# maxilevi/vits.cpp

Hardware: AMD Instinct MI355X
Metric: audio samples/sec end-to-end (ids -> fp32 PCM in HBM), vits-english architecture, batch=64 x 128 ids (higher is better)
Workload: dtype f32; 1 GPU; c3 b64x128 ref-mode f32 predicted-dur | vits-english = MMS-TTS arch, synthetic weights; batch_per_gpu=64, ids_per_utterance=128, parallelism=utterance-sharded x1

## Files before the change

vits.cpp_amd/csrc/abi_ops_common.h:

```cpp
#pragma once
#include <algorithm>
#include <cstdint>
#include <cstring>
#include <memory>
#include <string>
#include <vector>

#include "../../include/vits.h"
#include "abi_internal.h"
#include "engine.h"

namespace vits {
extern thread_local int g_op_out_fill;
extern thread_local int g_op_arith;

inline bool refuse(const std::string& why) {
    set_err(why);
    return false;
}

struct DevMem {
    void* p = nullptr;
    DevMem() = default;
    DevMem(const DevMem&) = delete;
    DevMem& operator=(const DevMem&) = delete;
    ~DevMem() {
        if (p) hipFree(p);
    }
    static bool ok(hipError_t e, const char* what) { return e == hipSuccess || refuse(what); }
    bool alloc(size_t bytes) { return ok(hipMalloc(&p, std::max<size_t>(bytes, 16)), "device allocation failed"); }
    bool fill(size_t bytes, int byte) { return alloc(bytes) && ok(hipMemset(p, byte, std::max<size_t>(bytes, 16)), "device allocation failed"); }
    bool put(const void* h, size_t bytes) { return h ? alloc(bytes) && ok(hipMemcpy(p, h, bytes, hipMemcpyHostToDevice), "device allocation failed") : fill(bytes, 0); }
    bool put_opt(const void* h, size_t bytes) { return !h || put(h, bytes); }
    bool get(void* h, size_t bytes) const { return ok(hipMemcpy(h, p, bytes, hipMemcpyDeviceToHost), "copy back failed"); }
    float* f() const { return static_cast<float*>(p); }
    uint16_t* h() const { return static_cast<uint16_t*>(p); }
    int* i() const { return static_cast<int*>(p); }
};

inline TensorRef tref(float* p, int channels, int stride) {
    TensorRef t;
    t.p = p;
    t.cs = stride;
    t.bs = (int64_t)channels * stride;
    return t;
}
inline bool lens_ok(const int32_t* lens, int batch, int t) {
    for (int b = 0; lens && b < batch; ++b)
        if (lens[b] < 0 || lens[b] > t) return false;
    return true;
}
inline bool shape_lens_ok(const int32_t* lens, int batch, int t, int t_stride) { return batch >= 1 && t >= 1 && t_stride >= t && lens_ok(lens, batch, t); }

inline bool finish(hipError_t e, const std::string& what = "") {
    if (e == hipSuccess) e = hipDeviceSynchronize();
    if (e == hipSuccess) return true;
    set_err(what.empty() ? std::string(hipGetErrorString(e)) : what + ": " + hipGetErrorString(e));
    return false;
}

inline bool stage_rows(DevMem& dst, const float* src, int batch, int rows, int64_t src_pitch, int64_t pitch, const int32_t* lens, int t) {
    std::vector<float> h((size_t)batch * rows * pitch);
    std::memset(h.data(), 0xFF, h.size() * 4);
    for (int b = 0; src && b < batch; ++b)
        for (int c = 0; c < rows; ++c)
            std::memcpy(&h[((size_t)b * rows + c) * pitch], src + ((size_t)b * rows + c) * src_pitch, sizeof(float) * (size_t)(lens ? lens[b] : t));
    return dst.put(h.data(), h.size() * 4);
}
inline bool unstage_rows(const DevMem& src, float* dst, int batch, int rows, int64_t pitch, int64_t dst_pitch, int t) {
    return DevMem::ok(hipMemcpy2D(dst, (size_t)dst_pitch * 4, src.p, (size_t)pitch * 4, (size_t)t * 4, (size_t)batch * rows, hipMemcpyDeviceToHost), "copy back failed");
}
inline bool stage_group8(DevMem& dst, const float* src, int batch, int channels, int64_t src_pitch, int64_t pitch, const int32_t* lens, int t) {
    std::vector<float> h((size_t)batch * channels * pitch);
    std::memset(h.data(), 0xFF, h.size() * 4);
    for (int b = 0; b < batch; ++b)
        for (int c = 0; c < channels; ++c) {
            const float* s = src + ((size_t)b * channels + c) * src_pitch;
            float* g = &h[((size_t)b * channels + (size_t)(c / 8) * 8) * pitch + (c & 7)];
            for (int n = 0, len = lens ? lens[b] : t; n < len; ++n) g[(size_t)n * 8] = s[n];
        }
    return dst.put(h.data(), h.size() * 4);
}
template <class T>
inline bool unstage_group8(const DevMem& src, T* dst, int batch, int channels, int64_t pitch, int64_t dst_pitch, int t) {
    std::vector<T> h((size_t)batch * channels * pitch);
    if (!src.get(h.data(), h.size() * sizeof(T))) return false;
    for (int b = 0; b < batch; ++b)
        for (int c = 0; c < channels; ++c) {
            const T* g = &h[((size_t)b * channels + (size_t)(c / 8) * 8) * pitch + (c & 7)];
            T* d = dst + ((size_t)b * channels + c) * dst_pitch;
            for (int n = 0; n < t; ++n) d[n] = g[(size_t)n * 8];
        }
    return true;
}

struct OpKnobs {
    KernelKnobs k;
    KernelKnobsScope scope;
    OpKnobs() : k(kernel_knobs()), scope(&k) {
        k.no_tile_map = getenv("VITS_NO_TILE_MAP") != nullptr;
        k.tile_map = getenv("VITS_TILE_MAP") != nullptr;
    }
};
struct OpTileMaps {
    TileMapSet set;
    std::vector<std::unique_ptr<DevMem>> mem;
    bool add(const int32_t* len_in, const int32_t* len_out, int batch, int t_in, int t_out, int width, bool convt) {
        const KernelKnobs& kn = kernel_knobs();
        if (kn.no_tile_map || set.find(width, convt)) return true;
        std::vector<int> la(batch, t_in), lb(batch, t_out);
        if (len_in) la.assign(len_in, len_in + batch);
        if (len_out) lb.assign(len_out, len_out + batch);
        if (!kn.tile_map && !tile_map_needed(la.data(), lb.data(), batch, t_in, t_out, width, convt)) return true;
        std::vector<TileEntry> e((size_t)tile_map_count(la.data(), lb.data(), batch, width, convt) + 1);
        const int64_t n = tile_map_fill(la.data(), lb.data(), batch, width, convt, e.data());
        mem.emplace_back(new DevMem);
        if (!mem.back()->put(e.data(), e.size() * sizeof(TileEntry))) return false;
        return set.add(TileMapRef{static_cast<const TileEntry*>(mem.back()->p), (int)n, width, convt}) || refuse("too many tile widths for one length vector");
    }
    bool add_conv(const int32_t* len_in, const int32_t* len_out, int batch, int t_in, int t_out, bool convt) {
        return add(len_in, len_out, batch, t_in, t_out, tile_shape(TILE_128x128).bn(), convt) && add(len_in, len_out, batch, t_in, t_out, tile_shape(TILE_64x256).bn(), convt);
    }
};

struct Conv {
    PackedConv pc;
    DevMem w, wl, w16, b;
};
inline bool upload_conv(Conv& c, const float* w, const float* bias, size_t bias_n, int cout, int cin, int taps, int epi, int ct_stride, int arith, bool l16_always = false) {
    PackedConv& pc = c.pc;
    const ConvPackDims pd = conv_pack_dims(cout, cin, taps, epi, ct_stride);
    pc.cin = cin, pc.cout = cout, pc.kt = pd.kt, pc.epi = epi, pc.ct_stride = ct_stride;
    pc.rows = pd.rows, pc.mtiles_used = pd.mtiles_used, pc.mtiles = pd.mtiles, pc.nchunks = pd.nchunks;
    if (bias) {
        if (!c.b.put(bias, bias_n * 4)) return false;
        pc.bias = c.b.f();
    }
    if (arith != VITS_ARITH_F32) {
        const std::vector<uint16_t> p16 = pack_conv_weights16(w, cout, cin, taps, epi, ct_stride, arith);
        if (!c.w16.put(p16.data(), p16.size() * 2)) return false;
        pc.wp16 = c.w16.h(), pc.bytes16 = (int64_t)p16.size() * 2;
        return true;
    }
    const std::vector<float> packed = pack_conv_weights(w, cout, cin, taps, epi, ct_stride, &pc.rows, &pc.mtiles_used, &pc.mtiles, &pc.nchunks);
    if (!c.w.put(packed.data(), packed.size() * 4)) return false;
    pc.wp = c.w.f(), pc.bytes = (int64_t)packed.size() * 4;
    if (l16_always || conv_lat16_candidate(epi, taps, cin)) {
        const std::vector<float> pl = repack_conv_weights_l16(packed, pc.mtiles, pc.nchunks, pc.kt);
        if (!c.wl.put(pl.data(), pl.size() * 4)) return false;
        pc.wp_l16 = c.wl.f();
    }
    return true;
}

inline size_t group16_bytes(int batch, int cin, int t) { return (size_t)batch * ((cin + 7) / 8 + 1) * round_up(t, 8) * 8 * 2; }
inline hipError_t conv_transparent(const PackedConv& w, const ConvCall& c, int arith, const DevMem& x16, size_t nan_bytes = 0) {
    if (arith == VITS_ARITH_F32) return launch_conv(w, c, nullptr);
    Ref16 r;
    r.p = x16.h(), r.ts = round_up(c.t_in, 8), r.bs = (int64_t)((w.cin + 7) / 8) * r.ts * 8;
    if (nan_bytes && hipMemsetAsync(x16.p, 0xFF, nan_bytes, nullptr) != hipSuccess) return hipErrorUnknown;
    const hipError_t e = launch_to_group16(c.x, c.len_in, c.batch, w.cin, c.t_in, c.pre_act ? c.slope : 1.0f, r, arith, nullptr);
    if (e != hipSuccess) return e;
    Conv16Call q;
    q.x = r, q.len_in = c.len_in, q.len_out = c.len_out, q.spk = c.spk, q.batch = c.batch, q.t_in = c.t_in, q.t_out = c.t_out, q.dil = c.dil, q.pad_l = c.pad_l;
    q.post_act = c.post_act, q.post_slope = c.post_slope, q.scale = c.scale, q.scale_div = c.scale_div, q.ct_crop = c.ct_crop, q.tile = c.tile;
    q.y = c.y, q.res = c.res, q.acc = c.acc;
    return launch_conv16(w, q, arith, nullptr);
}
}
```

vits.cpp_amd/csrc/kernel_common.h:

```cpp
#pragma once

#include <cstdint>

#include "tile_map.h"

#ifdef __HIPCC__
namespace vits {

typedef float floatx16 __attribute__((ext_vector_type(16)));
typedef float float4v __attribute__((ext_vector_type(4)));
typedef float float2v __attribute__((ext_vector_type(2)));
typedef int int4v __attribute__((ext_vector_type(4)));
typedef int int2v __attribute__((ext_vector_type(2)));
typedef _Float16 half8 __attribute__((ext_vector_type(8)));
typedef __bf16 bf16x8 __attribute__((ext_vector_type(8)));
typedef _Float16 half2v __attribute__((ext_vector_type(2)));
typedef __bf16 bf2v __attribute__((ext_vector_type(2)));

template <bool BF>
__device__ __forceinline__ unsigned pack16(float a, float b) {
    float2v f = {a, b};
    if constexpr (BF) return __builtin_bit_cast(unsigned, __builtin_convertvector(f, bf2v));
    else return __builtin_bit_cast(unsigned, __builtin_convertvector(f, half2v));
}
template <bool BF>
__device__ __forceinline__ float unpack16(unsigned short h) {
    if constexpr (BF) return __builtin_bit_cast(float, (unsigned)h << 16);
    else return (float)__builtin_bit_cast(_Float16, h);
}
template <bool BF>
__device__ __forceinline__ floatx16 mfma16(int4v a, int4v b, floatx16 c) {
    if constexpr (BF) return __builtin_amdgcn_mfma_f32_32x32x16_bf16(__builtin_bit_cast(bf16x8, a), __builtin_bit_cast(bf16x8, b), c, 0, 0, 0);
    else return __builtin_amdgcn_mfma_f32_32x32x16_f16(__builtin_bit_cast(half8, a), __builtin_bit_cast(half8, b), c, 0, 0, 0);
}

struct TileCoord {
    int b, t0, len_a, len_b;
};
__device__ __forceinline__ TileCoord tile_coord(const TileEntry* map, int bx, int bz, int bn, const int* len_a, const int* len_b, int max_a, int max_b) {
    TileCoord c;
    if (map) {
        const int4v e = *reinterpret_cast<const int4v*>(map + bx);
        c.b = e.x, c.t0 = e.y, c.len_a = e.z, c.len_b = e.w;
    } else {
        c.b = bz, c.t0 = bx * bn;
        c.len_a = len_a ? len_a[bz] : max_a;
        c.len_b = len_b ? len_b[bz] : max_b;
    }
    return c;
}

__device__ __forceinline__ __amdgpu_buffer_rsrc_t stream_rsrc(const void* base) {
    return __builtin_amdgcn_make_buffer_rsrc(const_cast<void*>(base), 0, 0x7fffffff, 0x00020000);
}
template <typename V>
__device__ __forceinline__ V load_frag(__amdgpu_buffer_rsrc_t wrsrc, int voff, int step, int sbase = 0) {
    return __builtin_bit_cast(V, __builtin_amdgcn_raw_buffer_load_b128(wrsrc, voff, sbase + step * 1024, 0));
}

__device__ __forceinline__ int64_t group_off(int ch0, int ts, int t) { return ((int64_t)(ch0 >> 3) * ts + t) * 8 + (ch0 & 7); }

__device__ __forceinline__ float scale_or_div(float v, float scale, int scale_div) { return scale_div ? v / scale : v * scale; }

__device__ __forceinline__ void group_add_scale(float (&v)[4], float4v a, float scale, int scale_div) {
#pragma unroll
    for (int e = 0; e < 4; ++e) {
        v[e] = a[e] + v[e];
        v[e] = scale_or_div(v[e], scale, scale_div);
    }
}
template <bool BF>
__device__ __forceinline__ void group_store(float (&v)[4], float* yg, int64_t go, uint16_t* y16, int y16_ts, float y16_slope, int ch0, int t) {
    if (yg) *reinterpret_cast<float4v*>(yg + go) = float4v{v[0], v[1], v[2], v[3]};
    if (y16) {
#pragma unroll
        for (int e = 0; e < 4; ++e) v[e] = fmaxf(v[e], v[e] * y16_slope);
        int2v w2;
        w2.x = (int)pack16<BF>(v[0], v[1]);
        w2.y = (int)pack16<BF>(v[2], v[3]);
        *reinterpret_cast<int2v*>(y16 + group_off(ch0, y16_ts, t)) = w2;
    }
}

__device__ __forceinline__ float ggml_table_lookup(const uint16_t* tab, float x) {
    const uint16_t i = __builtin_bit_cast(uint16_t, (_Float16)x);
    return (float)__builtin_bit_cast(_Float16, tab[i]);
}
__device__ __forceinline__ float gelu_erf(float x) { return 0.5f * x * (1.0f + erff(x * 0.70710678118654752440f)); }
__device__ __forceinline__ float gelu_op(float x, const uint16_t* gelu_tab) { return gelu_tab ? ggml_table_lookup(gelu_tab, x) : gelu_erf(x); }

}
#endif
```

vits.cpp_amd/csrc/kernels.h:

```cpp
#pragma once
#include <hip/hip_runtime.h>
#include <hip/hip_ext.h>

#include <algorithm>
#include <atomic>
#include <cstdint>
#include <cstdlib>
#include <string>
#include <vector>

#include "tile_map.h"

struct vits_edges_desc;

namespace vits {

struct KernelKnobs {
    int narrow_tiles = 64;
    int tile128 = 1;
    int min_blocks = 0;
    bool no_narrow = false;
    int narrow_k1 = 1 << 30;
    int nbuf = 0;
    bool no_oneshot = false;
    int db_min = 1;
    int t16_tile0 = 0;
    bool no_convt16s = false;
    bool convt16s_all = false;
    bool no_convt16l = false;
    bool no_att_lat = false;
    bool att_valu = false;
    int att_nw = 0;
    int att_short = 512;
    int ln_tw = 32;
    bool rbb_c128 = true;
    int rbb_c64k11 = -1;
    int rbb_stream_tiles = -1;
    int rbb_stream_min_blocks = 1536;
    int fuse16_maxc = 256;
    bool fuse32_c128 = true;
    int wn16_ncw = 1;
    int flow_ncw = 2;
    int convt16_r128 = 0;
    int convt16_split_max = 64;
    bool no_rbb_group3_c64 = false;
    bool no_rbb_group3 = false;
    bool no_rb_sum3_f32 = false;
    bool rb_sum3_in_order = false;
    bool rb_sum3_block_only = false;
    bool no_rb_sum3 = false;
    int rb16_narrow_max = 128;
    int flow_narrow_max = 96;
    bool no_ln_fuse = false;
    bool no_dds_lat = false;
    int dds_lat_max_blocks = 96;
    bool no_dp_det_fuse = false;
    int dp_det_lat_max_blocks = 96;
    int lat16h_group_shape = 21;
    bool no_lat16h_group = false;
    bool no_lat16h_pre = false;
    bool no_lat16h = false;
    int lat16h_max_tiles = 2048;
    int lat16h_max_tiles_c128 = 0;
    int lat16h_shape = 21;
    bool no_lat16 = false;
    int lat16_max_waves = 768;
    bool no_tile_map = false;
    bool tile_map = false;
    static KernelKnobs from_env() {
        KernelKnobs k;
        auto num = [](const char* name, int& v) {
            if (const char* e = getenv(name)) v = atoi(e);
        };
        auto flag = [](const char* name, bool& v) { v = getenv(name) != nullptr; };
        num("VITS_NARROW_TILES", k.narrow_tiles);
        flag("VITS_NO_DDS_LAT", k.no_dds_lat);
        flag("VITS_NO_LN_FUSE", k.no_ln_fuse);
        flag("VITS_NO_RB_SUM3", k.no_rb_sum3);
        flag("VITS_RB_SUM3_BLOCK_ONLY", k.rb_sum3_block_only);
        flag("VITS_RB_SUM3_IN_ORDER", k.rb_sum3_in_order);
        flag("VITS_NO_RB_SUM3_F32", k.no_rb_sum3_f32);
        flag("VITS_NO_RBB_GROUP3", k.no_rbb_group3);
        flag("VITS_NO_RBB_GROUP3_C64", k.no_rbb_group3_c64);
        num("VITS_DDS_LAT_MAX_BLOCKS", k.dds_lat_max_blocks);
        flag("VITS_NO_DP_DET_FUSE", k.no_dp_det_fuse);
        num("VITS_DP_DET_LAT_MAX_BLOCKS", k.dp_det_lat_max_blocks);
        num("VITS_TILE128", k.tile128);
        num("VITS_MIN_BLOCKS", k.min_blocks);
        flag("VITS_NO_NARROW", k.no_narrow);
        num("VITS_NARROW_K1", k.narrow_k1);
        num("VITS_NBUF", k.nbuf);
        flag("VITS_NO_ONESHOT", k.no_oneshot);
        num("VITS_DB_MIN", k.db_min);
        num("VITS_T16_TILE0", k.t16_tile0);
        flag("VITS_NO_CONVT16S", k.no_convt16s);
        flag("VITS_CONVT16S_ALL", k.convt16s_all);
        flag("VITS_NO_CONVT16L", k.no_convt16l);
        flag("VITS_ATT_VALU", k.att_valu);
        flag("VITS_NO_ATT_LAT", k.no_att_lat);
        num("VITS_ATT_NW", k.att_nw);
        num("VITS_ATT_SHORT", k.att_short);
        num("VITS_LN_TW", k.ln_tw);
        if (const char* e = getenv("VITS_RBB_C128")) k.rbb_c128 = atoi(e) != 0;
        num("VITS_RBB_C64K11", k.rbb_c64k11);
        num("VITS_RBB_STREAM_TILES", k.rbb_stream_tiles);
        num("VITS_RBB_STREAM_MIN_BLOCKS", k.rbb_stream_min_blocks);
        num("VITS_FUSE16_MAXC", k.fuse16_maxc);
        if (const char* e = getenv("VITS_FUSE32_C128")) k.fuse32_c128 = atoi(e) != 0;
        num("VITS_WN16_NCW", k.wn16_ncw);
        num("VITS_FLOW_NCW", k.flow_ncw);
        num("VITS_FLOW_NARROW_MAX", k.flow_narrow_max);
        num("VITS_RB16_NARROW_MAX", k.rb16_narrow_max);
        num("VITS_CONVT16_SPLIT_MAX", k.convt16_split_max);
        num("VITS_CONVT16_R128", k.convt16_r128);
        flag("VITS_NO_LAT16", k.no_lat16);
        flag("VITS_NO_LAT16H", k.no_lat16h);
        flag("VITS_NO_LAT16H_PRE", k.no_lat16h_pre);
        flag("VITS_NO_LAT16H_GROUP", k.no_lat16h_group);
        num("VITS_LAT16H_GROUP_SHAPE", k.lat16h_group_shape);
        num("VITS_LAT16H_MAX_TILES", k.lat16h_max_tiles);
        num("VITS_LAT16H_MAX_TILES_C128", k.lat16h_max_tiles_c128);
        num("VITS_LAT16H_SHAPE", k.lat16h_shape);
        num("VITS_LAT16_MAX_WAVES", k.lat16_max_waves);
        flag("VITS_NO_TILE_MAP", k.no_tile_map);
        flag("VITS_TILE_MAP", k.tile_map);
        return k;
    }
};
namespace detail {
inline thread_local const KernelKnobs* tl_kernel_knobs = nullptr;
}
inline const KernelKnobs& kernel_knobs() {
    if (detail::tl_kernel_knobs) return *detail::tl_kernel_knobs;
    static const KernelKnobs process_default = KernelKnobs::from_env();
    return process_default;
}
struct KernelKnobsScope {
    const KernelKnobs* prev;
    explicit KernelKnobsScope(const KernelKnobs* k) : prev(detail::tl_kernel_knobs) { detail::tl_kernel_knobs = k; }
    ~KernelKnobsScope() { detail::tl_kernel_knobs = prev; }
    KernelKnobsScope(const KernelKnobsScope&) = delete;
    KernelKnobsScope& operator=(const KernelKnobsScope&) = delete;
};

constexpr int kSmallGridBlocks = 512;
inline std::atomic<uint64_t>& tile_map_launches() {
    static std::atomic<uint64_t> n{0};
    return n;
}
inline void tile_map_launch_issued() { tile_map_launches().fetch_add(1, std::memory_order_relaxed); }
inline const TileMapRef* tile_map_for(const TileMapSet* maps, int width, bool convt, int64_t dense_blocks) {
    const KernelKnobs& kn = kernel_knobs();
    if (!maps || kn.no_tile_map) return nullptr;
    const TileMapRef* m = maps->find(width, convt);
    if (!m || !m->dev) return nullptr;
    return kn.tile_map || dense_blocks >= kSmallGridBlocks ? m : nullptr;
}

struct BigLdsOnce {
    std::atomic<uint64_t> mask{0};
    static uint64_t bit() {
        int d = 0;
        (void)hipGetDevice(&d);
        return 1ull << (d & 63);
    }
    bool needed() const { return !(mask.load(std::memory_order_acquire) & bit()); }
    void done() { mask.fetch_or(bit(), std::memory_order_release); }
    hipError_t raise(const void* kernel, size_t lds, int limit = 160 * 1024) {
        if (lds <= 64 * 1024 || !needed()) return hipSuccess;
        if (hipError_t e = hipFuncSetAttribute(kernel, hipFuncAttributeMaxDynamicSharedMemorySize, limit)) return e;
        done();
        return hipSuccess;
    }
};

struct LaunchTimer {
    hipEvent_t start = nullptr, stop = nullptr;
    int launches = 0;
};
inline thread_local LaunchTimer vits_launch_timer;
#define VITS_KLAUNCH(kernel, grid, block, lds, stream, ...)                                                          \
    do {                                                                                                            \
        ::vits::LaunchTimer& lt_ = ::vits::vits_launch_timer;                                                       \
        if (lt_.start && lt_.launches++ == 0)                                                                       \
            hipExtLaunchKernelGGL(kernel, grid, block, lds, stream, lt_.start, lt_.stop, 0, __VA_ARGS__);           \
        else                                                                                                        \
            hipLaunchKernelGGL(kernel, grid, block, lds, stream, __VA_ARGS__);                                      \
    } while (0)

template <auto Kernel, int LIMIT = 160 * 1024, class... A>
inline hipError_t launch_lds(dim3 grid, dim3 block, size_t lds, hipStream_t s, const A&... args) {
    static BigLdsOnce once;
    if (hipError_t e = once.raise(reinterpret_cast<const void*>(Kernel), lds, LIMIT)) return e;
    VITS_KLAUNCH(Kernel, grid, block, lds, s, args...);
    return hipGetLastError();
}

#ifdef __HIPCC__
__device__ __forceinline__ float wavenet_gate(float a, float s) { return tanhf(a) * (1.0f / (1.0f + expf(-s))); }
#endif

struct TensorRef {
    float* p = nullptr;
    int64_t bs = 0;
    int32_t cs = 0;
};

enum ConvEpilogue : int { EPI_STD = 0, EPI_GATE = 1, EPI_CONVT = 2 };
enum ConvTile : int {
    TILE_128x128 = 0,
    TILE_64x256 = 1,
    TILE_32x256 = 2,
    TILE_64x64 = 3,
    TILE_32x64 = 4,
    TILE_NARROW = 5,
    TILE_LAT16 = 6
};

struct PackedConv {
    float* wp = nullptr;
    float* bias = nullptr;
    int64_t bias_rs = 0;
    int cin = 0, cout = 0, kt = 0;
    int rows = 0;
    int mtiles = 0;
    int mtiles_used = 0;
    int nchunks = 0;
    int epi = EPI_STD;
    int ct_stride = 0;
    int64_t bytes = 0;
    uint16_t* wp16 = nullptr;
    float* wp_l16 = nullptr;
    int64_t bytes16 = 0;
    uint16_t* wps = nullptr;
    int64_t bytes_s = 0;
};

struct Ref16 {
    uint16_t* p = nullptr;
    int64_t bs = 0;
    int32_t ts = 0;
};

struct Split3Ref {
    uint16_t* p = nullptr;
    int64_t bs = 0;
    int64_t ps = 0;
    int32_t ts = 0;
};

struct ConvCall {
    TensorRef x, y, res, acc;
    const int* len_in = nullptr;
    const int* len_out = nullptr;
    const int* spk = nullptr;
    int batch = 1;
    int t_in = 0, t_out = 0;
    int64_t sum_in = -1, sum_out = -1;
    int dil = 1, pad_l = 0;
    int pre_act = 0;
    float slope = 0.f;
    int post_act = 0;
    float post_slope = 0.f;
    float* y2 = nullptr;
    float scale = 1.f;
    int scale_div = 0;
    int ct_crop = 0;
    int tile = -1;
    const TileMapSet* maps = nullptr;
    const float *ln_gamma = nullptr, *ln_beta = nullptr;
    float ln_eps = 0.f;
    TensorRef ln_out;
    Split3Ref xs3, ys3;
    float ys3_slope = 1.f;
};
bool conv_split_candidate(int epi, int kt, int cin, int cout);
bool pack_conv_weights_split(const float* w, int cout, int cin, int k, std::vector<uint16_t>& out);
bool conv_split_supported(const PackedConv& w, int dil);
// ... 486 lines not shown
```

vits.cpp_amd/csrc/rbblock32.hip:

```cpp
#include <hip/hip_runtime.h>

#include <atomic>
#include <cstdint>
#include <cstdlib>

#include "../../include/vits.h"
#include "kernel_common.h"
#include "kernels.h"

namespace vits {


struct RbBlock32Params {
    const float* x;
    int64_t x_bs;
    int x_cs;
    const float* w1[3];
    const float* w2[3];
    const float* b1[3];
    const float* b2[3];
    const int* lens;
    const TileEntry* tmap;
    int tmax;
    float slope;
    float* y;
    int64_t y_bs;
    int y_cs;
    const float* acc;
    int64_t a_bs;
    int a_cs;
    float scale;
    int scale_div;
    int post_act;
    float post_slope;
};

template <int C, int NR>
__global__ __launch_bounds__(256, C >= 64 ? 2 : 3) void rbblock32_kernel(const RbBlock32Params p) {
    constexpr int KT = 3, D0 = 1, D1 = 3, D2 = 5;
    constexpr int NCH = C / 32, WM = C / 32, WN = 4 / WM;
    constexpr RbBlock32Geom GEO = rbblock32_geom(C, NR);
    constexpr int W = GEO.w, P2 = GEO.p2, H = GEO.h, BO = GEO.bo;
    constexpr int PADX = GEO.padx;
    constexpr int PITCH = GEO.pitch;
    constexpr int TOTAL = NCH * KT * 4;
    static_assert(BO > 0, "tile too narrow");
    extern __shared__ __attribute__((aligned(16))) float tile[];
    float* lbias = tile + C * PITCH;

    const int tid = threadIdx.x, lane = tid & 63, wid = tid >> 6;
    const int wm = wid / WN, wn = wid % WN;
    const TileCoord tc = tile_coord(p.tmap, blockIdx.x, blockIdx.y, BO, p.lens, nullptr, p.tmax, 0);
    const int b = tc.b;
    const int len = tc.len_a;
    const int t0 = tc.t0;
    if (t0 >= len) return;
    const int krow = lane >> 5, col = lane & 31;
    const int u0 = wn * (NR * 32) + col;
    const int tg0 = t0 - H;
    typedef const __attribute__((address_space(3))) float* LdsF;
    const float* xb = p.x + (int64_t)b * p.x_bs;

    floatx16 yv[NR];
#pragma unroll
    for (int nr = 0; nr < NR; ++nr) {
        const int t = tg0 + u0 + 32 * nr;
        const bool inside = t >= 0 && t < len;
#pragma unroll
        for (int r = 0; r < 16; ++r) {
            const int row = wm * 32 + (r >> 2) * 8 + krow * 4 + (r & 3);
            yv[nr][r] = inside ? xb[(int64_t)row * p.x_cs + t] : 0.f;
        }
    }
    for (int i = tid; i < 6 * C; i += 256) {
        const int pi = i / (2 * C), r = i - pi * 2 * C;
        lbias[i] = r < C ? p.b1[pi][r] : p.b2[pi][r - C];
    }
    for (int i = tid; i < C * (PITCH - W); i += 256) {
        const int row = i / (PITCH - W), m = i - row * (PITCH - W);
        tile[row * PITCH + (m < PADX ? m : W + m)] = 0.f;
    }
    auto write_tile = [&](const floatx16 (&src)[NR], const float* bias_p) __attribute__((always_inline)) {
#pragma unroll
        for (int nr = 0; nr < NR; ++nr) {
            const int u = u0 + 32 * nr, t = tg0 + u;
            const bool inside = t >= 0 && t < len;
#pragma unroll
            for (int r = 0; r < 16; ++r) {
                const int row = wm * 32 + (r >> 2) * 8 + krow * 4 + (r & 3);
                float v = src[nr][r];
                if (bias_p) v = v + bias_p[row];
                v = fmaxf(v, v * p.slope);
                tile[row * PITCH + PADX + u] = inside ? v : 0.f;
            }
        }
        asm volatile("s_waitcnt lgkmcnt(0)" ::: "memory");
    };

    floatx16 acc[NR];
    float4v ring[4];
    const int wvoff = (int)(((size_t)wm * TOTAL * 64 + lane) * 16);
    auto load_a = [&](const float* wp, int step) __attribute__((always_inline)) -> float4v {
        const __amdgpu_buffer_rsrc_t wrsrc = stream_rsrc(wp);
        return load_frag<float4v>(wrsrc, wvoff, step);
    };
    auto prefetch = [&](const float* wp) __attribute__((always_inline)) {
        ring[0] = load_a(wp, 0);
        ring[1] = load_a(wp, 1 < TOTAL ? 1 : 0);
    };
    auto conv = [&](const float* wp, const int off0, const int dstep) __attribute__((always_inline)) {
#pragma unroll
        for (int j = 0; j < NR; ++j)
#pragma unroll
            for (int r = 0; r < 16; ++r) acc[j][r] = 0.f;
        LdsF base = (LdsF)(tile + krow * PITCH + PADX + u0 + off0);
#pragma unroll
        for (int c = 0; c < NCH; ++c) {
#pragma unroll
            for (int j = 0; j < KT; ++j) {
                LdsF xj = base + (c * 32) * PITCH + j * dstep;
#pragma unroll
                for (int p4 = 0; p4 < 4; ++p4) {
                    const int s = (c * KT + j) * 4 + p4;
                    ring[(s + 2) & 3] = load_a(wp, s + 2 < TOTAL ? s + 2 : TOTAL - 1);
                    __builtin_amdgcn_sched_barrier(0);
                    const float4v a4 = ring[s & 3];
#pragma unroll
                    for (int q = 0; q < 4; ++q) {
                        const int pair = p4 * 4 + q;
                        float bv[NR];
#pragma unroll
                        for (int nr = 0; nr < NR; ++nr) bv[nr] = xj[(2 * pair) * PITCH + nr * 32];
#pragma unroll
                        for (int nr = 0; nr < NR; ++nr) acc[nr] = __builtin_amdgcn_mfma_f32_32x32x2f32(a4[q], bv[nr], acc[nr], 0, 0, 0);
                    }
                }
            }
        }
    };

    auto pair = [&](const int pi, const int dil, const bool last) __attribute__((always_inline)) {
        conv(p.w1[pi], -P2 * dil, dil);
        prefetch(p.w2[pi]);
        __syncthreads();
        write_tile(acc, lbias + pi * 2 * C);
        __syncthreads();
        conv(p.w2[pi], -P2, 1);
        if (!last) prefetch(p.w1[pi + 1]);
#pragma unroll
        for (int nr = 0; nr < NR; ++nr)
#pragma unroll
            for (int r = 0; r < 16; ++r) {
                const int row = wm * 32 + (r >> 2) * 8 + krow * 4 + (r & 3);
                const float v = acc[nr][r] + lbias[pi * 2 * C + C + row];
                yv[nr][r] = yv[nr][r] + v;
            }
        if (!last) {
            __syncthreads();
            write_tile(yv, nullptr);
            __syncthreads();
        }
    };

    prefetch(p.w1[0]);
    __syncthreads();
    write_tile(yv, nullptr);
    __syncthreads();
    pair(0, D0, false);
    pair(1, D1, false);
    pair(2, D2, true);

    {
        float* yb = p.y + (int64_t)b * p.y_bs;
        const float* ab = p.acc ? p.acc + (int64_t)b * p.a_bs : nullptr;
#pragma unroll
        for (int nr = 0; nr < NR; ++nr) {
            const int u = u0 + 32 * nr, t = tg0 + u;
            if (u < H || u >= H + BO || t >= len) continue;
            float av[16];
            if (ab) {
#pragma unroll
                for (int r = 0; r < 16; ++r) {
                    const int row = wm * 32 + (r >> 2) * 8 + krow * 4 + (r & 3);
                    av[r] = ab[(int64_t)row * p.a_cs + t];
                }
            }
#pragma unroll
            for (int r = 0; r < 16; ++r) {
                const int row = wm * 32 + (r >> 2) * 8 + krow * 4 + (r & 3);
                float v = yv[nr][r];
                if (ab) {
                    v = av[r] + v;
                    v = scale_or_div(v, p.scale, p.scale_div);
                }
                if (p.post_act == 2) v = fmaxf(v, v * p.post_slope);
                yb[(int64_t)row * p.y_cs + t] = v;
            }
        }
    }
}

hipError_t launch_rbblock32(const PackedConv* const* c1, const PackedConv* const* c2, const RbBlock32Call& c, hipStream_t s) {
    const int C = c1[0]->cin, kt = c1[0]->kt;
    RbBlock32Params p;
    for (int i = 0; i < 3; ++i) {
        if (!c1[i]->wp || !c2[i]->wp || !c1[i]->bias || !c2[i]->bias || c1[i]->cin != C || c1[i]->cout != C || c2[i]->cin != C || c2[i]->cout != C || c1[i]->kt != kt ||
            c2[i]->kt != kt)
            return hipErrorInvalidValue;
        p.w1[i] = c1[i]->wp;
        p.w2[i] = c2[i]->wp;
        p.b1[i] = c1[i]->bias;
        p.b2[i] = c2[i]->bias;
    }
    const RbBlock32Plan l = plan_rbblock32(C, kt, c.batch, c.tmax);
    if (!l.ok || !c.x.p || !c.y.p || c.x.p == c.y.p) return hipErrorInvalidValue;
    p.x = c.x.p, p.x_bs = c.x.bs, p.x_cs = c.x.cs, p.lens = c.lens, p.tmax = c.tmax, p.slope = c.slope, p.y = c.y.p, p.y_bs = c.y.bs, p.y_cs = c.y.cs;
    p.acc = c.acc.p, p.a_bs = c.acc.bs, p.a_cs = c.acc.cs, p.scale = c.scale, p.scale_div = c.scale_div, p.post_act = c.post_act;
    p.post_slope = c.post_slope;
    static_assert(rbblock32_exists(32, rbblock32_nr(32)) && rbblock32_exists(64, rbblock32_nr(64)), "the planner's predicate");
    const TileMapRef* tm = tile_map_for(c.maps, rbblock32_geom(C, l.nr).bo, false, (int64_t)l.gx * l.gy);
    p.tmap = tm ? tm->dev : nullptr;
    if (tm && tm->n == 0) return hipSuccess;
    if (tm) tile_map_launch_issued();
    const dim3 grid(tm ? tm->n : l.gx, tm ? 1 : l.gy), block(l.block);
    if (C == 32) return launch_lds<&rbblock32_kernel<32, rbblock32_nr(32)>>(grid, block, l.lds, s, p);
    return launch_lds<&rbblock32_kernel<64, rbblock32_nr(64)>>(grid, block, l.lds, s, p);
}

}
```

vits.cpp_amd/csrc/rbpair32.hip:

```cpp
#include <hip/hip_runtime.h>

#include <atomic>
#include <cstdint>
#include <cstdlib>

#include "../../include/vits.h"
#include "kernel_common.h"
#include "kernels.h"

namespace vits {


struct RbPair32Params {
    const float* x;
    int64_t x_bs;
    int x_cs;
    const float *w1, *w2;
    const float *b1, *b2;
    const int* lens;
    const TileEntry* tmap;
    int tmax;
    float slope;
    float* y;
    int64_t y_bs;
    int y_cs;
    const float* acc;
    int64_t a_bs;
    int a_cs;
    float scale;
    int scale_div;
    int post_act;
    float post_slope;
};

template <int KT, int DIL, int C>
__global__ __launch_bounds__(256, C >= 128 ? 2 : 3) void rbpair32_kernel(const RbPair32Params p) {
    constexpr int NCH = C / 32;
    constexpr RbPair32Geom GEO = rbpair32_geom(KT, DIL, C);
    constexpr int WN = GEO.wn, NR = GEO.nr;
    constexpr int BO = GEO.bo;
    constexpr int P2 = (KT - 1) / 2, P1 = (KT - 1) * DIL / 2;
    constexpr int XWP = GEO.xwp;
    constexpr int XW4 = XWP / 4;
    constexpr int TWP = GEO.twp;
    constexpr int TOTAL = NCH * KT * 4;
    static_assert(TWP <= XWP, "the t tile takes the x tile's place");
    extern __shared__ __attribute__((aligned(16))) float lds[];
    float* xs = lds;
    float* ts = lds;

    const int tid = threadIdx.x, lane = tid & 63, wid = tid >> 6;
    const TileCoord tc = tile_coord(p.tmap, blockIdx.x, blockIdx.y, BO, p.lens, nullptr, p.tmax, 0);
    const int b = tc.b;
    const int len = tc.len_a;
    const int t0 = tc.t0;
    if (t0 >= len) return;
    const int wm = wid / WN, wn = wid % WN;
    const int cb = wn * (NR * 32);
    const int krow = lane >> 5;

    const int tx0 = t0 - P2 - P1;
    const int ts0 = tx0 & ~3;
    const int shift = tx0 - ts0;
    const float* xb = p.x + (int64_t)b * p.x_bs;
    {
        const __amdgpu_buffer_rsrc_t xrsrc = stream_rsrc(xb);
        const int tlast = (len - 1) & ~3;
        constexpr int N4 = C * XW4;
        constexpr int NI = (N4 + 63) / 64;
#pragma unroll
        for (int n0 = 0; n0 < NI; n0 += 4) {
            const int n = n0 + wid;
            if (n < NI) {
                int g = n * 64 + lane;
                g = g < N4 ? g : N4 - 1;
                const int r = g / XW4, c4 = g - r * XW4;
                int t = ts0 + 4 * c4;
                t = t < 0 ? 0 : (t > tlast ? tlast : t);
                __builtin_amdgcn_raw_ptr_buffer_load_lds(xrsrc, (__attribute__((address_space(3))) void*)(xs + n * 256), 16, (r * p.x_cs + t) * 4, 0, 0, 0);
            }
        }
    }
    float bias1[16], bias2[16];
#pragma unroll
    for (int r = 0; r < 16; ++r) {
        const int row = wm * 32 + (r >> 2) * 8 + krow * 4 + (r & 3);
        bias1[r] = p.b1[row];
        bias2[r] = p.b2[row];
    }
    asm volatile("s_waitcnt vmcnt(0)" ::: "memory");
    __syncthreads();
    {
        float4v* x4 = reinterpret_cast<float4v*>(xs);
        constexpr int N4 = C * XW4;
        for (int g = tid; g < N4; g += 256) {
            const int r = g / XW4, c4 = g - r * XW4;
            const int t = ts0 + 4 * c4;
            float4v v = x4[g];
#pragma unroll
            for (int e = 0; e < 4; ++e) {
                float u = v[e];
                u = fmaxf(u, u * p.slope);
                v[e] = (t + e < 0 || t + e >= len) ? 0.f : u;
            }
            x4[g] = v;
        }
    }
    __syncthreads();

    floatx16 acc[NR];
    typedef const __attribute__((address_space(3))) float* LdsF;

    auto conv = [&](const float* wp, LdsF base, const int pitch, const int dstep) __attribute__((always_inline)) {
#pragma unroll
        for (int j = 0; j < NR; ++j)
#pragma unroll
            for (int r = 0; r < 16; ++r) acc[j][r] = 0.f;
        const __amdgpu_buffer_rsrc_t wrsrc = stream_rsrc(wp);
        const int wvoff = (int)(((size_t)wm * TOTAL * 64 + lane) * 16);
        auto load_a = [&](int step) __attribute__((always_inline)) -> float4v {
            return load_frag<float4v>(wrsrc, wvoff, step);
        };
        float4v ring[4];
        ring[0] = load_a(0);
        ring[1] = load_a(1 < TOTAL ? 1 : 0);
#pragma unroll
        for (int c = 0; c < NCH; ++c) {
#pragma unroll
            for (int j = 0; j < KT; ++j) {
                LdsF xj = base + (c * 32) * pitch + j * dstep;
#pragma unroll
                for (int p4 = 0; p4 < 4; ++p4) {
                    const int s = (c * KT + j) * 4 + p4;
                    ring[(s + 2) & 3] = load_a(s + 2 < TOTAL ? s + 2 : TOTAL - 1);
                    __builtin_amdgcn_sched_barrier(0);
                    const float4v a4 = ring[s & 3];
#pragma unroll
                    for (int q = 0; q < 4; ++q) {
                        const int pair = p4 * 4 + q;
                        float bv[NR];
#pragma unroll
                        for (int nr = 0; nr < NR; ++nr) bv[nr] = xj[(2 * pair) * pitch + nr * 32];
#pragma unroll
                        for (int nr = 0; nr < NR; ++nr) acc[nr] = __builtin_amdgcn_mfma_f32_32x32x2f32(a4[q], bv[nr], acc[nr], 0, 0, 0);
                    }
                }
            }
        }
    };

    conv(p.w1, (LdsF)(xs + krow * XWP + shift + cb + (lane & 31)), XWP, DIL);
    __syncthreads();

#pragma unroll
    for (int nr = 0; nr < NR; ++nr) {
        const int i = cb + nr * 32 + (lane & 31);
        const int tm = t0 - P2 + i;
        const bool inside = tm >= 0 && tm < len;
#pragma unroll
        for (int r = 0; r < 16; ++r) {
            const int row = wm * 32 + (r >> 2) * 8 + krow * 4 + (r & 3);
            float v = acc[nr][r] + bias1[r];
            v = fmaxf(v, v * p.slope);
            ts[row * TWP + i] = inside ? v : 0.f;
        }
    }
    __syncthreads();

    conv(p.w2, (LdsF)(ts + krow * TWP + cb + (lane & 31)), TWP, 1);

    {
        float* yb = p.y + (int64_t)b * p.y_bs;
        const float* ab = p.acc ? p.acc + (int64_t)b * p.a_bs : nullptr;
#pragma unroll
        for (int nr = 0; nr < NR; ++nr) {
            const int o = cb + nr * 32 + (lane & 31);
            const int t = t0 + o;
            if (o >= BO || t >= len) continue;
            float rv[16];
#pragma unroll
            for (int r = 0; r < 16; ++r) {
                const int row = wm * 32 + (r >> 2) * 8 + krow * 4 + (r & 3);
                rv[r] = xb[(int64_t)row * p.x_cs + t];
            }
#pragma unroll
            for (int r = 0; r < 16; ++r) {
                const int row = wm * 32 + (r >> 2) * 8 + krow * 4 + (r & 3);
                float v = acc[nr][r] + bias2[r];
                v = rv[r] + v;
                if (ab) {
                    v = ab[(int64_t)row * p.a_cs + t] + v;
                    v = scale_or_div(v, p.scale, p.scale_div);
                }
                if (p.post_act == 2) v = fmaxf(v, v * p.post_slope);
                yb[(int64_t)row * p.y_cs + t] = v;
            }
        }
    }
}

template <int KT, int DIL, int C>
static hipError_t launch_rb32(const RbPair32Params& p, const LaunchGrid& l, hipStream_t s) {
    static_assert(rbpair32_exists(KT, DIL, C), "the planner would never ask for it");
    return launch_lds<&rbpair32_kernel<KT, DIL, C>>(dim3(l.gx, l.gy), dim3(l.block), l.lds, s, p);
}

template <int KT, int C>
static hipError_t launch_rb32_dil(int dil, const RbPair32Params& p, const LaunchGrid& l, hipStream_t s) {
    switch (dil) {
        case 1: return launch_rb32<KT, 1, C>(p, l, s);
        case 3: return launch_rb32<KT, 3, C>(p, l, s);
        case 5: return launch_rb32<KT, 5, C>(p, l, s);
        default: return hipErrorInvalidValue;
    }
}

template <int C>
static hipError_t launch_rb32_kt(int kt, int dil, const RbPair32Params& p, const LaunchGrid& l, hipStream_t s) {
    switch (kt) {
        case 3: return launch_rb32_dil<3, C>(dil, p, l, s);
        case 7: return launch_rb32_dil<7, C>(dil, p, l, s);
        case 11: return launch_rb32_dil<11, C>(dil, p, l, s);
        default: return hipErrorInvalidValue;
    }
}

hipError_t launch_rbpair32(const PackedConv& c1, const PackedConv& c2, const RbPair32Call& c, hipStream_t s) {
    LaunchGrid l = plan_rbpair32(c1.cin, c1.kt, c.dil, c.batch, c.tmax);
    if (!c1.wp || !c2.wp || c1.cin != c1.cout || c2.cin != c1.cout || c2.cout != c1.cout || c1.kt != c2.kt || !l.ok ||
        !c1.bias || !c2.bias || c.x.p == c.y.p)
        return hipErrorInvalidValue;
    if ((c.x.cs & 3) || (c.x.bs & 3) || (reinterpret_cast<uintptr_t>(c.x.p) & 15)) return hipErrorInvalidValue;
    RbPair32Params p;
    p.x = c.x.p, p.x_bs = c.x.bs, p.x_cs = c.x.cs, p.w1 = c1.wp, p.w2 = c2.wp, p.b1 = c1.bias, p.b2 = c2.bias, p.lens = c.lens, p.tmax = c.tmax;
    p.slope = c.slope, p.y = c.y.p, p.y_bs = c.y.bs, p.y_cs = c.y.cs, p.acc = c.acc.p, p.a_bs = c.acc.bs, p.a_cs = c.acc.cs, p.scale = c.scale;
    p.scale_div = c.scale_div, p.post_act = c.post_act, p.post_slope = c.post_slope;
    const TileMapRef* tm = tile_map_for(c.maps, rbpair32_geom(c1.kt, c.dil, c1.cin).bo, false, (int64_t)l.gx * l.gy);
    p.tmap = tm ? tm->dev : nullptr;
    if (tm) {
        if (tm->n == 0) return hipSuccess;
        l.gx = tm->n, l.gy = 1;
        tile_map_launch_issued();
    }
    if (c1.cin == 32) return launch_rb32_kt<32>(c1.kt, c.dil, p, l, s);
    if (c1.cin == 64) return launch_rb32_kt<64>(c1.kt, c.dil, p, l, s);
    return launch_rb32_dil<3, 128>(c.dil, p, l, s);
}

}
```

Before: 51.14 million samples/s.

## Add fast interior paths and DPP-transposed vector epilogues to rb32 resblock kernels

For tiles that lie fully inside the valid length, the rbpair32 and rbblock32 kernels now take branch-free paths. These cover the leaky-ReLU LDS pass and the tile write. The epilogue uses DPP quad transposes so each lane can issue 128-bit row loads and stores of residual, accumulator and output in place of scalar strided accesses. The aim is to cut global memory transaction count and per-element bounds checks in the resblock epilogues. It adds register pressure and code paths gated by alignment checks, plus an env knob and optional phase-timing stamps.

New measurement: 51.54 million samples/s, median of 6. About the same (+0.8%).

```diff
diff --git a/vits.cpp_amd/csrc/abi_ops_common.h b/vits.cpp_amd/csrc/abi_ops_common.h
--- a/vits.cpp_amd/csrc/abi_ops_common.h
+++ b/vits.cpp_amd/csrc/abi_ops_common.h
@@ -100,6 +100,7 @@
     OpKnobs() : k(kernel_knobs()), scope(&k) {
         k.no_tile_map = getenv("VITS_NO_TILE_MAP") != nullptr;
         k.tile_map = getenv("VITS_TILE_MAP") != nullptr;
+        k.rb32_plain = getenv("VITS_RB32_PLAIN") != nullptr;
     }
 };
 struct OpTileMaps {
diff --git a/vits.cpp_amd/csrc/kernel_common.h b/vits.cpp_amd/csrc/kernel_common.h
--- a/vits.cpp_amd/csrc/kernel_common.h
+++ b/vits.cpp_amd/csrc/kernel_common.h
@@ -58,6 +58,59 @@
     return __builtin_bit_cast(V, __builtin_amdgcn_raw_buffer_load_b128(wrsrc, voff, sbase + step * 1024, 0));
 }
 
+__device__ __forceinline__ void quad_transpose4(float& v0, float& v1, float& v2, float& v3, bool odd1, bool odd2) {
+    {
+        float s01 = odd1 ? v0 : v1, s23 = odd1 ? v2 : v3;
+        s01 = __builtin_bit_cast(float, __builtin_amdgcn_mov_dpp(__builtin_bit_cast(int, s01), 0xB1, 0xF, 0xF, true));
+        s23 = __builtin_bit_cast(float, __builtin_amdgcn_mov_dpp(__builtin_bit_cast(int, s23), 0xB1, 0xF, 0xF, true));
+        if (odd1) { v0 = s01; v2 = s23; } else { v1 = s01; v3 = s23; }
+    }
+    {
+        float s02 = odd2 ? v0 : v2, s13 = odd2 ? v1 : v3;
+        s02 = __builtin_bit_cast(float, __builtin_amdgcn_mov_dpp(__builtin_bit_cast(int, s02), 0x4E, 0xF, 0xF, true));
+        s13 = __builtin_bit_cast(float, __builtin_amdgcn_mov_dpp(__builtin_bit_cast(int, s13), 0x4E, 0xF, 0xF, true));
+        if (odd2) { v0 = s02; v1 = s13; } else { v2 = s02; v3 = s13; }
+    }
+}
+
+typedef float float4u __attribute__((ext_vector_type(4), aligned(4)));
+typedef float float2u __attribute__((ext_vector_type(2), aligned(4)));
+__device__ __forceinline__ float4v row_load4(const float* base, int voff, int soff) {
+    const float4u t = *reinterpret_cast<const float4u*>(reinterpret_cast<const char*>(base) + soff + (unsigned)voff);
+    return float4v{t[0], t[1], t[2], t[3]};
+}
+__device__ __forceinline__ float2v row_load2(const float* base, int voff, int soff) {
+    const float2u t = *reinterpret_cast<const float2u*>(reinterpret_cast<const char*>(base) + soff + (unsigned)voff);
+    return float2v{t[0], t[1]};
+}
+__device__ __forceinline__ void row_store4(float4v v, float* base, int voff, int soff) {
+    *reinterpret_cast<float4u*>(reinterpret_cast<char*>(base) + soff + (unsigned)voff) = float4u{v[0], v[1], v[2], v[3]};
+}
+__device__ __forceinline__ void row_store2(float2v v, float* base, int voff, int soff) {
+    *reinterpret_cast<float2u*>(reinterpret_cast<char*>(base) + soff + (unsigned)voff) = float2u{v[0], v[1]};
+}
+enum : int {
+    RB32_FAST_RELU = 1,
+    RB32_FAST_WIDE = 2,
+    RB32_FAST_TWRITE = 4
+};
+inline bool rb32_wide_ok(const void* base, int64_t bs, int cs, int rows) {
+    return !(cs & 3) && !(bs & 3) && !(reinterpret_cast<uintptr_t>(base) & 15) && cs > 0 && (int64_t)rows * cs * 4 < (int64_t)0x7fff0000;
+}
+
+#ifdef VITS_PHASE_TIMING
+__device__ unsigned long long vits_rb32_phase[8 * 65536];
+#define RB32_STAMP(k)                                                                                     \
+    do {                                                                                                  \
+        if (threadIdx.x == 0) {                                                                           \
+            const unsigned lin = blockIdx.x + gridDim.x * blockIdx.y;                                     \
+            if (lin < 65536) vits_rb32_phase[8 * lin + (k)] = __builtin_readcyclecounter();               \
+        }                                                                                                 \
+    } while (0)
+#else
+#define RB32_STAMP(k)
+#endif
+
 __device__ __forceinline__ int64_t group_off(int ch0, int ts, int t) { return ((int64_t)(ch0 >> 3) * ts + t) * 8 + (ch0 & 7); }
 
 __device__ __forceinline__ float scale_or_div(float v, float scale, int scale_div) { return scale_div ? v / scale : v * scale; }
diff --git a/vits.cpp_amd/csrc/kernels.h b/vits.cpp_amd/csrc/kernels.h
--- a/vits.cpp_amd/csrc/kernels.h
+++ b/vits.cpp_amd/csrc/kernels.h
@@ -66,6 +66,7 @@
     bool no_lat16 = false;
     int lat16_max_waves = 768;
     bool no_tile_map = false;
+    bool rb32_plain = false;
     bool tile_map = false;
     static KernelKnobs from_env() {
         KernelKnobs k;
@@ -124,6 +125,7 @@
         num("VITS_LAT16_MAX_WAVES", k.lat16_max_waves);
         flag("VITS_NO_TILE_MAP", k.no_tile_map);
         flag("VITS_TILE_MAP", k.tile_map);
+        flag("VITS_RB32_PLAIN", k.rb32_plain);
         return k;
     }
 };
diff --git a/vits.cpp_amd/csrc/rbblock32.hip b/vits.cpp_amd/csrc/rbblock32.hip
--- a/vits.cpp_amd/csrc/rbblock32.hip
+++ b/vits.cpp_amd/csrc/rbblock32.hip
@@ -3,6 +3,7 @@
 #include <atomic>
 #include <cstdint>
 #include <cstdlib>
+#include <type_traits>
 
 #include "../../include/vits.h"
 #include "kernel_common.h"
@@ -33,6 +34,7 @@
     int scale_div;
     int post_act;
     float post_slope;
+    int fast;
 };
 
 template <int C, int NR>
@@ -55,6 +57,7 @@
     const int len = tc.len_a;
     const int t0 = tc.t0;
     if (t0 >= len) return;
+    RB32_STAMP(0);
     const int krow = lane >> 5, col = lane & 31;
     const int u0 = wn * (NR * 32) + col;
     const int tg0 = t0 - H;
@@ -80,7 +83,22 @@
         const int row = i / (PITCH - W), m = i - row * (PITCH - W);
         tile[row * PITCH + (m < PADX ? m : W + m)] = 0.f;
     }
+    const bool all_in = (p.fast & RB32_FAST_TWRITE) && tg0 >= 0 && tg0 + W <= len;
     auto write_tile = [&](const floatx16 (&src)[NR], const float* bias_p) __attribute__((always_inline)) {
+        if (all_in) {
+#pragma unroll
+            for (int nr = 0; nr < NR; ++nr) {
+                const int u = u0 + 32 * nr;
+#pragma unroll
+                for (int r = 0; r < 16; ++r) {
+                    const int row = wm * 32 + (r >> 2) * 8 + krow * 4 + (r & 3);
+                    float v = src[nr][r];
+                    if (bias_p) v = v + bias_p[row];
+                    v = fmaxf(v, v * p.slope);
+                    tile[row * PITCH + PADX + u] = v;
+                }
+            }
+        } else
 #pragma unroll
         for (int nr = 0; nr < NR; ++nr) {
             const int u = u0 + 32 * nr, t = tg0 + u;
@@ -166,11 +184,79 @@
     __syncthreads();
     write_tile(yv, nullptr);
     __syncthreads();
+    RB32_STAMP(1);
     pair(0, D0, false);
+    RB32_STAMP(2);
     pair(1, D1, false);
+    RB32_STAMP(3);
     pair(2, D2, true);
-
+    RB32_STAMP(4);
+
+    RB32_STAMP(5);
+#ifdef VITS_RB32_NOEPI
     {
+        float keep = 0.f;
+#pragma unroll
+        for (int nr = 0; nr < NR; ++nr)
+#pragma unroll
+            for (int r = 0; r < 16; ++r) keep += yv[nr][r];
+        if (keep == 123.456f) p.y[tid] = keep;
+        return;
+    }
+#endif
+    static_assert(H % 4 == 0 && BO % 4 == 0, "a quad of columns is owned whole or not at all");
+    if ((p.fast & RB32_FAST_WIDE) && t0 + BO <= len) {
+        float* yb = p.y + (int64_t)b * p.y_bs;
+        const float* ab = p.acc ? p.acc + (int64_t)b * p.a_bs : nullptr;
+        const int qi = lane & 3, cq = col & ~3;
+        const bool odd1 = lane & 1, odd2 = lane & 2;
+        const int wmu = __builtin_amdgcn_readfirstlane(wm);
+        const int uq = wn * (NR * 32) + cq;
+        const int yvoff = ((krow * 4 + qi) * p.y_cs + tg0 + uq) * 4, avoff = ((krow * 4 + qi) * p.a_cs + tg0 + uq) * 4;
+        auto owned = [&](int nr) __attribute__((always_inline)) -> bool { return uq + 32 * nr >= H && uq + 32 * nr < H + BO; };
+        auto epilogue = [&](auto sum_c, auto act_c) __attribute__((always_inline)) {
+            constexpr int SUM = decltype(sum_c)::value;
+            constexpr bool ACT = decltype(act_c)::value;
+            float4v aq[2][4];
+            auto load_sum = [&](int nr, float4v* dst) __attribute__((always_inline)) {
+#pragma unroll
+                for (int g = 0; g < 4; ++g) {
+                    if (owned(nr)) dst[g] = row_load4(ab, avoff + nr * 128, (wmu * 32 + 8 * g) * p.a_cs * 4);
+                    else dst[g] = float4v{0.f, 0.f, 0.f, 0.f};
+                }
+            };
+            if (SUM) load_sum(0, aq[0]);
+#pragma unroll
+            for (int nr = 0; nr < NR; ++nr) {
+                if (SUM && nr + 1 < NR) load_sum(nr + 1, aq[(nr + 1) & 1]);
+                __builtin_amdgcn_sched_barrier(0);
+                const bool own = owned(nr);
+#pragma unroll
+                for (int g = 0; g < 4; ++g) {
+                    float v[4] = {yv[nr][4 * g], yv[nr][4 * g + 1], yv[nr][4 * g + 2], yv[nr][4 * g + 3]};
+                    quad_transpose4(v[0], v[1], v[2], v[3], odd1, odd2);
+#pragma unroll
+                    for (int e = 0; e < 4; ++e) {
+                        float u = v[e];
+                        if (SUM) {
+                            u = aq[nr & 1][g][e] + u;
+                            u = SUM == 2 ? u / p.scale : u * p.scale;
+                        }
+                        if (ACT) u = fmaxf(u, u * p.post_slope);
+                        v[e] = u;
+                    }
+                    if (own) row_store4(float4v{v[0], v[1], v[2], v[3]}, yb, yvoff + nr * 128, (wmu * 32 + 8 * g) * p.y_cs * 4);
+                }
+            }
+        };
+        auto with_act = [&](auto sum_c) __attribute__((always_inline)) {
+            if (p.post_act == 2) epilogue(sum_c, std::true_type{});
+            else epilogue(sum_c, std::false_type{});
+        };
+        if (!ab) with_act(std::integral_constant<int, 0>{});
+        else if (!p.scale_div) with_act(std::integral_constant<int, 1>{});
+        else with_act(std::integral_constant<int, 2>{});
+    } else {
         float* yb = p.y + (int64_t)b * p.y_bs;
         const float* ab = p.acc ? p.acc + (int64_t)b * p.a_bs : nullptr;
 #pragma unroll
@@ -198,6 +284,7 @@
             }
         }
     }
+    RB32_STAMP(6);
 }
 
 hipError_t launch_rbblock32(const PackedConv* const* c1, const PackedConv* const* c2, const RbBlock32Call& c, hipStream_t s) {
@@ -217,6 +304,11 @@
     p.x = c.x.p, p.x_bs = c.x.bs, p.x_cs = c.x.cs, p.lens = c.lens, p.tmax = c.tmax, p.slope = c.slope, p.y = c.y.p, p.y_bs = c.y.bs, p.y_cs = c.y.cs;
     p.acc = c.acc.p, p.a_bs = c.acc.bs, p.a_cs = c.acc.cs, p.scale = c.scale, p.scale_div = c.scale_div, p.post_act = c.post_act;
     p.post_slope = c.post_slope;
+    const bool aligned = rb32_wide_ok(c.y.p, c.y.bs, c.y.cs, C) && (!c.acc.p || rb32_wide_ok(c.acc.p, c.acc.bs, c.acc.cs, C));
+    p.fast = kernel_knobs().rb32_plain ? 0 : RB32_FAST_TWRITE | (aligned ? RB32_FAST_WIDE : 0);
+#ifdef VITS_RB32_FAST_MASK
+    p.fast &= VITS_RB32_FAST_MASK;
+#endif
     static_assert(rbblock32_exists(32, rbblock32_nr(32)) && rbblock32_exists(64, rbblock32_nr(64)), "the planner's predicate");
     const TileMapRef* tm = tile_map_for(c.maps, rbblock32_geom(C, l.nr).bo, false, (int64_t)l.gx * l.gy);
     p.tmap = tm ? tm->dev : nullptr;
diff --git a/vits.cpp_amd/csrc/rbpair32.hip b/vits.cpp_amd/csrc/rbpair32.hip
--- a/vits.cpp_amd/csrc/rbpair32.hip
+++ b/vits.cpp_amd/csrc/rbpair32.hip
@@ -3,6 +3,7 @@
 #include <atomic>
 #include <cstdint>
 #include <cstdlib>
+#include <type_traits>
 
 #include "../../include/vits.h"
 #include "kernel_common.h"
@@ -31,6 +32,7 @@
     int scale_div;
     int post_act;
     float post_slope;
+    int fast;
 };
 
 template <int KT, int DIL, int C>
@@ -55,6 +57,7 @@
     const int len = tc.len_a;
     const int t0 = tc.t0;
     if (t0 >= len) return;
+    RB32_STAMP(0);
     const int wm = wid / WN, wn = wid % WN;
     const int cb = wn * (NR * 32);
     const int krow = lane >> 5;
@@ -90,7 +93,22 @@
     }
     asm volatile("s_waitcnt vmcnt(0)" ::: "memory");
     __syncthreads();
-    {
+    RB32_STAMP(1);
+#ifndef VITS_RB32_NORELU
+    if ((p.fast & RB32_FAST_RELU) && ts0 >= 0 && ts0 + XWP <= len) {
+        float4v* x4 = reinterpret_cast<float4v*>(xs);
+        constexpr int N4 = C * XW4;
+#pragma unroll
+        for (int g0 = 0; g0 < N4; g0 += 256) {
+            const int g = g0 + tid;
+            if (g0 + 256 <= N4 || g < N4) {
+                float4v v = x4[g];
+#pragma unroll
+                for (int e = 0; e < 4; ++e) v[e] = fmaxf(v[e], v[e] * p.slope);
+                x4[g] = v;
+            }
+        }
+    } else {
         float4v* x4 = reinterpret_cast<float4v*>(xs);
         constexpr int N4 = C * XW4;
         for (int g = tid; g < N4; g += 256) {
@@ -106,7 +124,9 @@
             x4[g] = v;
         }
     }
+#endif
     __syncthreads();
+    RB32_STAMP(2);
 
     floatx16 acc[NR];
     typedef const __attribute__((address_space(3))) float* LdsF;
@@ -151,6 +171,7 @@
 
     conv(p.w1, (LdsF)(xs + krow * XWP + shift + cb + (lane & 31)), XWP, DIL);
     __syncthreads();
+    RB32_STAMP(3);
 
 #pragma unroll
     for (int nr = 0; nr < NR; ++nr) {
@@ -166,10 +187,93 @@
         }
     }
     __syncthreads();
+    RB32_STAMP(4);
+
+    static_assert((BO & 3) == 0 || (BO & 3) == 2, "the cut quad moves two columns");
+    const bool wide = (p.fast & RB32_FAST_WIDE) && t0 + BO <= len;
+    const int qi = lane & 3, cq = (lane & 31) & ~3;
+    const bool odd1 = lane & 1, odd2 = lane & 2;
+    const int wmu = __builtin_amdgcn_readfirstlane(wm);
+    const int rvoff = ((krow * 4 + qi) * p.x_cs + t0 + cb + cq) * 4;
+    float4v rq[2][4];
+    auto quad_state = [&](int nr) __attribute__((always_inline)) -> int {
+        const int o = cb + nr * 32 + cq;
+        return o + 4 <= BO ? 2 : (o + 2 <= BO ? 1 : 0);
+    };
+    auto load_rows = [&](const float* rs, int voff, int cs, int nr, float4v* dst) __attribute__((always_inline)) {
+        const int st = quad_state(nr);
+#pragma unroll
+        for (int g = 0; g < 4; ++g) {
+            const int soff = (wmu * 32 + 8 * g) * cs * 4;
+            if (st == 2) dst[g] = row_load4(rs, voff + nr * 128, soff);
+            else if (st == 1) {
+                const float2v h = row_load2(rs, voff + nr * 128, soff);
+                dst[g] = float4v{h[0], h[1], 0.f, 0.f};
+            } else dst[g] = float4v{0.f, 0.f, 0.f, 0.f};
+        }
+    };
 
     conv(p.w2, (LdsF)(ts + krow * TWP + cb + (lane & 31)), TWP, 1);
-
+    RB32_STAMP(5);
+#ifdef VITS_RB32_NOEPI
     {
+        float keep = 0.f;
+#pragma unroll
+        for (int nr = 0; nr < NR; ++nr)
+#pragma unroll
+            for (int r = 0; r < 16; ++r) keep += acc[nr][r];
+        if (keep == 123.456f) p.y[tid] = keep;
+        return;
+    }
+#endif
+
+    if (wide) {
+        float* yb = p.y + (int64_t)b * p.y_bs;
+        const int yvoff = ((krow * 4 + qi) * p.y_cs + t0 + cb + cq) * 4;
+        const float* ab = p.acc ? p.acc + (int64_t)b * p.a_bs : nullptr;
+        const int avoff = ((krow * 4 + qi) * p.a_cs + t0 + cb + cq) * 4;
+        auto epilogue = [&](auto sum_c, auto act_c) __attribute__((always_inline)) {
+            constexpr int SUM = decltype(sum_c)::value;
+            constexpr bool ACT = decltype(act_c)::value;
+            float4v aq[4];
+            load_rows(xb, rvoff, p.x_cs, 0, rq[0]);
+#pragma unroll
+            for (int nr = 0; nr < NR; ++nr) {
+                if (nr + 1 < NR) load_rows(xb, rvoff, p.x_cs, nr + 1, rq[(nr + 1) & 1]);
+                if (SUM) load_rows(ab, avoff, p.a_cs, nr, aq);
+                __builtin_amdgcn_sched_barrier(0);
+                const int st = quad_state(nr);
+#pragma unroll
+                for (int g = 0; g < 4; ++g) {
+                    float v[4];
+#pragma unroll
+                    for (int e = 0; e < 4; ++e) v[e] = acc[nr][4 * g + e] + bias2[4 * g + e];
+                    quad_transpose4(v[0], v[1], v[2], v[3], odd1, odd2);
+                    const float4v r4 = rq[nr & 1][g];
+#pragma unroll
+                    for (int e = 0; e < 4; ++e) {
+                        float u = r4[e] + v[e];
+                        if (SUM) {
+                            u = aq[g][e] + u;
+                            u = SUM == 2 ? u / p.scale : u * p.scale;
+                        }
+                        if (ACT) u = fmaxf(u, u * p.post_slope);
+                        v[e] = u;
+                    }
+                    const int soff = (wmu * 32 + 8 * g) * p.y_cs * 4;
+                    if (st == 2) row_store4(float4v{v[0], v[1], v[2], v[3]}, yb, yvoff + nr * 128, soff);
+                    else if (st == 1) row_store2(float2v{v[0], v[1]}, yb, yvoff + nr * 128, soff);
+                }
+            }
+        };
+        auto with_act = [&](auto sum_c) __attribute__((always_inline)) {
+            if (p.post_act == 2) epilogue(sum_c, std::true_type{});
+            else epilogue(sum_c, std::false_type{});
+        };
+        if (!ab) with_act(std::integral_constant<int, 0>{});
+        else if (!p.scale_div) with_act(std::integral_constant<int, 1>{});
+        else with_act(std::integral_constant<int, 2>{});
+    } else {
         float* yb = p.y + (int64_t)b * p.y_bs;
         const float* ab = p.acc ? p.acc + (int64_t)b * p.a_bs : nullptr;
 #pragma unroll
@@ -197,6 +301,7 @@
             }
         }
     }
+    RB32_STAMP(6);
 }
 
 template <int KT, int DIL, int C>
@@ -235,6 +340,11 @@
     p.x = c.x.p, p.x_bs = c.x.bs, p.x_cs = c.x.cs, p.w1 = c1.wp, p.w2 = c2.wp, p.b1 = c1.bias, p.b2 = c2.bias, p.lens = c.lens, p.tmax = c.tmax;
     p.slope = c.slope, p.y = c.y.p, p.y_bs = c.y.bs, p.y_cs = c.y.cs, p.acc = c.acc.p, p.a_bs = c.acc.bs, p.a_cs = c.acc.cs, p.scale = c.scale;
     p.scale_div = c.scale_div, p.post_act = c.post_act, p.post_slope = c.post_slope;
+    const bool aligned = rb32_wide_ok(c.x.p, c.x.bs, c.x.cs, c1.cin) && rb32_wide_ok(c.y.p, c.y.bs, c.y.cs, c1.cin) && (!c.acc.p || rb32_wide_ok(c.acc.p, c.acc.bs, c.acc.cs, c1.cin));
+    p.fast = kernel_knobs().rb32_plain ? 0 : RB32_FAST_RELU | (aligned ? RB32_FAST_WIDE : 0);
+#ifdef VITS_RB32_FAST_MASK
+    p.fast &= VITS_RB32_FAST_MASK;
+#endif
     const TileMapRef* tm = tile_map_for(c.maps, rbpair32_geom(c1.kt, c.dil, c1.cin).bo, false, (int64_t)l.gx * l.gy);
     p.tmap = tm ? tm->dev : nullptr;
     if (tm) {
```
